# bacpop/sparrowhawk

Hardware: AMD Instinct MI355X
Metric: Gbases/s assembled, k=31 150bp reads (higher is better)
Workload: dtype u64

## Files before the change

### sparrowhawk_amd/csrc/graph_part.h

```cpp
#pragma once

struct MinScan {
    Nt32State first, last;
    uint32_t h_first, h_last;
    uint32_t min_wo_first;
    uint32_t min_wo_last;
    __device__ __forceinline__ uint32_t min_all() const { return min(min_wo_first, h_first); }
};

template <int W> __device__ __forceinline__ uint32_t km_base(const Kmer<W> &x, int k, int j) {
    return km_bits2<W>(x, 2 * (k - 1 - j));
}

template <int W> __device__ __forceinline__ MinScan km_min_scan(const Kmer<W> &x, int k, int gm) {
    MinScan r;
    Nt32State nt{0, 0};
    for (int j = 0; j < gm; j++) nt32_init_step(nt, km_base<W>(x, k, j), (unsigned)j);
    r.first = nt; r.h_first = nt32_canonical(nt);
    r.min_wo_first = 0xFFFFFFFFu; r.min_wo_last = r.h_first;
    const int w = k - gm + 1;
    uint32_t h = r.h_first;
    for (int q = 1; q < w; q++) {
        nt32_roll(nt, km_base<W>(x, k, q - 1), km_base<W>(x, k, q + gm - 1), (unsigned)gm);
        h = nt32_canonical(nt);
// ... 176 lines not shown
            uint32_t sz = gp_table_size(c);
            if (p >= GP) sz = 0;
            uint32_t si = sz, ci = c;
#pragma unroll
            for (int o = 1; o < 16; o <<= 1) {
                const uint32_t u = (uint32_t)__shfl_up((int)si, o), v = (uint32_t)__shfl_up((int)ci, o);
                if ((lane & 15) >= o) { si += u; ci += v; }
            }
            if (p < GP) { off[p] = run_off[e >> 4] + (si - sz); msk[p] = sz - 1u; roff[p] = run_roff[e >> 4] + (ci - c); }
        }
        for (int w = 0; w < 16; w++) { carry += wsum[w]; rcarry += rsum[w]; }
        __syncthreads();
    }
    if (threadIdx.x == 0) { *total = carry; roff[GP] = rcarry; }
}

__global__ __launch_bounds__(256) void k_gp_rows(const uint32_t *__restrict__ gp_of, uint32_t n,
                                                 const uint32_t *__restrict__ roff, uint32_t *__restrict__ cursor,
                                                 uint32_t *__restrict__ rows) {
    const int lane = threadIdx.x & 63;
    const uint32_t stride = gridDim.x * blockDim.x;
    const uint32_t n_round = (n + stride - 1) / stride * stride;
    for (uint32_t i = blockIdx.x * blockDim.x + threadIdx.x; i < n_round; i += stride) {
        const uint32_t p = i < n ? gp_of[i] : 0xFFFFFFFFu;
        const bool valid = p != 0xFFFFFFFFu;
        unsigned long long todo = __ballot(valid);
        int my_leader = lane; uint32_t rank = 0, gsize = 0;
        while (todo) {
            const int leader = __ffsll((long long)todo) - 1;
            const uint32_t lp = (uint32_t)__shfl((int)p, leader);
            const unsigned long long same = __ballot(p == lp) & todo;
            if (valid && p == lp) { my_leader = leader; rank = (uint32_t)__popcll(same & ((1ull << lane) - 1ull)); gsize = (uint32_t)__popcll(same); }
            todo &= ~same;
        }
        const uint32_t ro = valid ? roff[p] : 0u;
        uint32_t base = 0;
        if (valid && lane == my_leader) base = atomicAdd(&cursor[p], gsize);
        base = (uint32_t)__shfl((int)base, my_leader);
        if (valid) rows[ro + base + rank] = i;
    }
}

template <int W>
__global__ __launch_bounds__(256) void k_regroup_rows(KeyArr<W> keys, const uint32_t *__restrict__ cnt, const uint32_t *__restrict__ gp_of,
                                                      uint32_t *__restrict__ rows, uint32_t n, KeyArr<W> out_keys,
                                                      uint32_t *__restrict__ out_cnt, uint32_t *__restrict__ out_gp_of) {
    for (uint32_t r = blockIdx.x * blockDim.x + threadIdx.x; r < n; r += gridDim.x * blockDim.x) {
        const uint32_t i = rows[r];
        out_keys.store(r, keys.load(i));
        out_cnt[r] = cnt[i];
        out_gp_of[r] = gp_of[i];
        rows[r] = r;
    }
}

template <int W>
__device__ __forceinline__ uint32_t gt_lookup_in(const GraphTable &gt, const KeyArr<W> &keys, const Kmer<W> &q,
                                                 uint32_t p) {
    const uint64_t h = gt_hash<W>(q);
    const uint32_t fp = (uint32_t)(h >> 32);
    const unsigned long long base = gt.off[p];
    const uint32_t mask = gt.msk[p];
    uint32_t slot = (uint32_t)h & mask;
    for (uint32_t t = 0; t <= mask; t++) {
        const uint64_t e = gt.e[base + slot];
        if (e == EMPTY64) return NIL;
        if ((uint32_t)(e >> 32) == fp) {
            const uint32_t idx = (uint32_t)e;
            if (km_eq<W>(keys.load(idx), q)) return idx;
        }
        slot = (slot + 1) & mask;
    }
    return NIL;
}
template <int W>
__device__ __forceinline__ uint32_t gt_lookup(const GraphTable &gt, const KeyArr<W> &keys, const Kmer<W> &q, int k) {
    return gt_lookup_in<W>(gt, keys, q, gt_partition_of<W>(gt, q, k));
}

static constexpr uint32_t ADJ_LDS_SLOTS = 2048;
static constexpr uint32_t NB_MULTI = 0xFFFFFFFEu;
static constexpr uint32_t ADJ_LDS_SLOTS_RANGES = 4096;
static constexpr int ADJ_THREADS_RANGES = 512;

struct GpRows {
    const uint32_t *roff;
    const uint32_t *cnt;
    const uint32_t *rows;
    __device__ __forceinline__ uint32_t begin(uint32_t P) const { return roff[P]; }
    __device__ __forceinline__ uint32_t end(uint32_t P) const { return cnt ? roff[P] + cnt[P] : roff[P + 1]; }
    __device__ __forceinline__ uint32_t row(uint32_t r) const { return rows ? rows[r] : r; }
};

template <int W>
__device__ __forceinline__ Kmer<W> adj_candidate(const Kmer<W> &x, const Kmer<W> &rx, int k, uint32_t j, bool &o) {
    Kmer<W> s = x, rr = rx;
    if (j < 4) { km_push_back<W>(s, j, k); km_push_front<W>(rr, 3u - j, k); }
    else { km_push_front<W>(s, j - 4u, k); km_push_back<W>(rr, 3u - (j - 4u), k); }
    o = km_less<W>(rr, s);
    Kmer<W> c;
#pragma unroll
    for (int w = 0; w < W; w++) c.w[w] = o ? rr.w[w] : s.w[w];
    return c;
}

template <int W, uint32_t SLOTS, int NT>
__global__ __launch_bounds__(NT) void k_graph_local(KeyArr<W> keys, int k, GraphTable gt, GpRows gr,
                                                    uint8_t *__restrict__ adj, uint32_t *__restrict__ nb,
                                                    unsigned long long *__restrict__ queries, uint32_t *__restrict__ qcnt,
                                                    uint32_t *__restrict__ overflow, uint32_t lds_slots ,
                                                    uint8_t *__restrict__ alive, uint32_t *__restrict__ row_bits, uint32_t lowmask) {
    const unsigned gm = (unsigned)gt.gm;
    __shared__ uint2 lut[16];
    __shared__ uint64_t tab[SLOTS];
    __shared__ uint32_t tabi[W == 1 ? SLOTS : 1];
    __shared__ uint32_t q_fill;
    const uint32_t P = blockIdx.x;
    const bool ranges = gr.cnt != nullptr;
    const uint32_t r0 = gr.begin(P), r1 = gr.end(P);
    const uint32_t pmask = gt.msk[P];
    const bool in_lds = pmask < lds_slots;
    uint64_t *gtab = gt.e + gt.off[P];
    nt32_fill_lut(lut, gm);
    const Nt32State all_a = nt32_all_a(gt.gm);
    if (threadIdx.x == 0) q_fill = 0;
    constexpr bool KEYS_IN_LDS = W == 1;
    for (uint32_t t = threadIdx.x; t <= pmask; t += blockDim.x) {
        if (in_lds) tab[t] = EMPTY64;
        if (!in_lds || KEYS_IN_LDS) gtab[t] = EMPTY64;
    }
    __syncthreads();
    constexpr int KEEP = 4;
    static_assert(SLOTS <= 2u * KEEP * NT, "a partition whose table fits the LDS keeps its rows in registers");
    const bool keep = W <= 2 && (r1 - r0) <= (uint32_t)KEEP * NT;
    static_assert(KEEP == 4, "kept rows are four named registers");
    const uint32_t rt = r0 + threadIdx.x;
    const uint32_t i0 = (keep && rt < r1) ? gr.row(rt) : NIL, i1 = (keep && rt + NT < r1) ? gr.row(rt + NT) : NIL;
    const uint32_t i2 = (keep && rt + 2 * NT < r1) ? gr.row(rt + 2 * NT) : NIL, i3 = (keep && rt + 3 * NT < r1) ? gr.row(rt + 3 * NT) : NIL;
    const Kmer<W> k0 = i0 != NIL ? keys.load(i0) : km_zero<W>(), k1 = i1 != NIL ? keys.load(i1) : km_zero<W>();
    const Kmer<W> k2 = i2 != NIL ? keys.load(i2) : km_zero<W>(), k3 = i3 != NIL ? keys.load(i3) : km_zero<W>();
    auto kept_i = [=](uint32_t q) { return q == 0 ? i0 : (q == 1 ? i1 : (q == 2 ? i2 : i3)); };
    auto kept_key = [=](uint32_t q) {
        Kmer<W> r;
#pragma unroll
        for (int w = 0; w < W; w++) r.w[w] = q == 0 ? k0.w[w] : (q == 1 ? k1.w[w] : (q == 2 ? k2.w[w] : k3.w[w]));
        return r;
    };
    for (uint32_t r = r0 + threadIdx.x, q = 0; r < r1; r += blockDim.x, q++) {
        const uint32_t i = keep ? kept_i(q) : gr.row(r);
        const Kmer<W> key = keep ? kept_key(q) : keys.load(i);
        const uint64_t h = gt_hash<W>(key);
        const uint64_t entry = (h & 0xFFFFFFFF00000000ull) | (uint64_t)i;
        uint32_t slot = (uint32_t)h & pmask;
        bool done = false;
        for (uint32_t t = 0; t <= pmask; t++) {
            if (in_lds && KEYS_IN_LDS) {
                if (atomicCAS((unsigned long long *)&tab[slot], (unsigned long long)EMPTY64, (unsigned long long)key.w[0]) == EMPTY64) {
                    tabi[slot] = i; gtab[slot] = entry; done = true; break;
                }
            } else {
                unsigned long long *cell = in_lds ? (unsigned long long *)&tab[slot] : (unsigned long long *)&gtab[slot];
                if (atomicCAS(cell, (unsigned long long)EMPTY64, (unsigned long long)entry) == EMPTY64) { done = true; break; }
            }
            slot = (slot + 1) & pmask;
        }
        if (!done) *overflow = 1;
    }
    __syncthreads();
    if (ranges && threadIdx.x == NT - 1 && r1 > r0) {
        bool st = r0 == 0u;
        if (!st) st = ((km_min_scan_lut<W>(keys.load(r0 - 1u), k, gt.gm, lut, all_a).min_all() ^ P) & lowmask) != 0u;
        if (st) atomicOr(&row_bits[r0 >> 5], 1u << (r0 & 31u));
    }
    if (in_lds && !KEYS_IN_LDS) for (uint32_t t = threadIdx.x; t <= pmask; t += blockDim.x) gtab[t] = tab[t];
    {
        uint8_t *occ = gt.occ + (gt.off[P] >> 3);
        for (uint32_t t8 = threadIdx.x; t8 <= (pmask >> 3); t8 += blockDim.x) {
            uint32_t bits = 0;
#pragma unroll
            for (uint32_t b = 0; b < 8; b++) {
                const uint64_t e = in_lds ? tab[8u * t8 + b] : __hip_atomic_load(&gtab[8u * t8 + b], __ATOMIC_RELAXED, __HIP_MEMORY_SCOPE_AGENT);
                bits |= (e != EMPTY64 ? 1u : 0u) << b;
            }
            occ[t8] = (uint8_t)bits;
        }
    }
    unsigned long long *myq = queries + 8ull * r0;
    const int lane = threadIdx.x & 63;
    const uint32_t n_rows = r1 - r0;
    const uint32_t n_round = (n_rows + blockDim.x - 1) / blockDim.x * blockDim.x;
    for (uint32_t rr_ = threadIdx.x, q = 0; rr_ < n_round; rr_ += blockDim.x, q++) {
        const bool act = rr_ < n_rows;
        const uint32_t i = act ? (keep ? kept_i(q) : gr.row(r0 + rr_)) : 0u;
        Kmer<W> x = km_zero<W>(), rx = km_zero<W>();
        MinScan ms{};
        uint32_t out_b = 0, last_b = 0;
        if (act) {
            x = keep ? kept_key(q) : keys.load(i);
            rx = km_revcomp<W>(x, k);
            if (gt.scan) {
                const uint2 a = gt.scan[i], b = gt.scan[(size_t)gt.scan_n + i], c = gt.scan[2 * (size_t)gt.scan_n + i];
                ms.first.fh = a.x; ms.first.rh = a.y; ms.last.fh = b.x; ms.last.rh = b.y; ms.min_wo_first = c.x; ms.min_wo_last = c.y;
                ms.h_first = min(a.x, a.y); ms.h_last = min(b.x, b.y);
            } else ms = km_min_scan_lut<W>(x, k, gt.gm, lut, all_a);
            if (ranges && ((ms.min_all() & gt.gp_mask) != P)) *overflow = 2u;
            out_b = km_base<W>(x, k, k - (int)gm);
            last_b = km_base<W>(x, k, (int)gm - 1);
        }
        uint32_t a = 0, n_out = 0, n_in = 0, u_out = NIL, u_in = NIL;
#pragma unroll
        for (uint32_t j = 0; j < 8; j++) {
            bool remote = false; uint32_t p = 0, xowner = 0; bool cross = false;
            if (act) {
                const uint32_t hmin = j < 4 ? min(ms.min_wo_first, nt32_next_hash_lut(ms.last, out_b, j, lut))
                                            : min(ms.min_wo_last, nt32_prev_hash_lut(ms.first, j - 4u, last_b, lut));
                p = hmin & gt.gp_mask;
                if (gt.world > 1) { xowner = gt.owner_of(hmin); cross = xowner != gt.rank; }
                remote = cross || p != P || !in_lds;
                if (!remote) {
                    bool o; const Kmer<W> c = adj_candidate<W>(x, rx, k, j, o);
                    const uint64_t h = gt_hash<W>(c);
                    const uint32_t fp = (uint32_t)(h >> 32);
                    uint32_t slot = (uint32_t)h & pmask, idx = NIL;
                    for (uint32_t t = 0; t <= pmask; t++) {
                        const uint64_t e = tab[slot];
                        if (e == EMPTY64) break;
                        if constexpr (KEYS_IN_LDS) { if (e == c.w[0]) { idx = tabi[slot]; break; } }
                        else if ((uint32_t)(e >> 32) == fp && km_eq<W>(keys.load((uint32_t)e), c)) { idx = (uint32_t)e; break; }
                        slot = (slot + 1) & pmask;
                    }
                    (void)fp;
                    if (idx != NIL) {
                        a |= 1u << j;
                        if (j < 4) { n_out++; u_out = idx * 2u + (o ? 1u : 0u); }
                        else { n_in++; u_in = idx * 2u + (o ? 0u : 1u); }
                    }
                }
            }
            const unsigned long long m = __ballot(remote);
            if (m) {
                uint32_t base = 0;
                if (lane == 0) base = atomicAdd(&q_fill, (uint32_t)__popcll(m));
                base = (uint32_t)__shfl((int)base, 0);
                if (remote) myq[base + (uint32_t)__popcll(m & ((1ull << lane) - 1ull))] =
                    (unsigned long long)i | ((unsigned long long)j << 32) | ((unsigned long long)p << 35) |
                    (cross ? (1ull << 63) | ((unsigned long long)xowner << 52) : 0ull);
            }
        }
        if (act) {
            adj[i] = (uint8_t)a;
            if (alive) alive[i] = 1;
            uint2 v;
            v.x = n_out == 0 ? NIL : (n_out == 1 ? u_out : NB_MULTI);
            v.y = n_in == 0 ? NIL : (n_in == 1 ? u_in : NB_MULTI);
            *reinterpret_cast<uint2 *>(nb + 2ull * i) = v;
        }
    }
    __syncthreads();
    if (threadIdx.x == 0) qcnt[P] = q_fill;
}

template <int W>
__global__ __launch_bounds__(256) void k_graph_remote(KeyArr<W> keys, int k, GraphTable gt, GpRows gr,
                                                      const unsigned long long *__restrict__ queries,
                                                      const uint32_t *__restrict__ qcnt,
                                                      uint8_t *__restrict__ adj, uint32_t *__restrict__ nb) {
    const uint32_t P = blockIdx.x;
    const unsigned long long *myq = queries + 8ull * gr.begin(P);
    const uint32_t nq = qcnt[P];
    constexpr int U = W <= 2 ? 4 : (W <= 4 ? 2 : 1);
    for (uint32_t t0 = threadIdx.x; t0 < nq; t0 += blockDim.x * U) {
        unsigned long long q[U]; bool live[U];
#pragma unroll
        for (int u = 0; u < U; u++) {
            const uint32_t t = t0 + (uint32_t)u * blockDim.x;
            q[u] = t < nq ? myq[t] : ~0ull;
            live[u] = !(q[u] >> 63);
        }
        Kmer<W> x[U]; unsigned long long tbase[U]; uint32_t tmask[U];
#pragma unroll
        for (int u = 0; u < U; u++) {
            const uint32_t i = (uint32_t)q[u], p = (uint32_t)(q[u] >> 35) & 0x1FFFFu;
            x[u] = live[u] ? keys.load(i) : km_zero<W>();
            tbase[u] = live[u] ? gt.off[p] : 0ull;
            tmask[u] = live[u] ? gt.msk[p] : 0u;
        }
        Kmer<W> c[U]; bool o[U]; uint32_t fp[U], slot[U]; uint64_t e[U];
#pragma unroll
        for (int u = 0; u < U; u++) {
            const uint32_t j = (uint32_t)(q[u] >> 32) & 7u;
            const Kmer<W> rx = km_revcomp<W>(x[u], k);
            c[u] = adj_candidate<W>(x[u], rx, k, j, o[u]);
            const uint64_t h = gt_hash<W>(c[u]);
            fp[u] = (uint32_t)(h >> 32); slot[u] = (uint32_t)h & tmask[u];
        }
        bool taken[U];
#pragma unroll
        for (int u = 0; u < U; u++) {
            const unsigned long long s = tbase[u] + slot[u];
            taken[u] = live[u] && ((gt.occ[s >> 3] >> (s & 7u)) & 1u);
        }
#pragma unroll
        for (int u = 0; u < U; u++) e[u] = taken[u] ? gt.e[tbase[u] + slot[u]] : EMPTY64;
        Kmer<W> cand[U]; bool want[U];
#pragma unroll
        for (int u = 0; u < U; u++) {
            want[u] = e[u] != EMPTY64 && (uint32_t)(e[u] >> 32) == fp[u];
            cand[u] = want[u] ? keys.load((uint32_t)e[u]) : km_zero<W>();
        }
#pragma unroll
        for (int u = 0; u < U; u++) {
            if (!live[u]) continue;
            uint32_t idx = NIL;
            if (want[u] && km_eq<W>(cand[u], c[u])) idx = (uint32_t)e[u];
            else if (e[u] != EMPTY64) {
                uint32_t s = (slot[u] + 1u) & tmask[u];
                for (uint32_t t = 1; t <= tmask[u]; t++) {
                    const uint64_t ee = gt.e[tbase[u] + s];
                    if (ee == EMPTY64) break;
                    if ((uint32_t)(ee >> 32) == fp[u] && km_eq<W>(keys.load((uint32_t)ee), c[u])) { idx = (uint32_t)ee; break; }
                    s = (s + 1u) & tmask[u];
                }
            }
            if (idx == NIL) continue;
            const uint32_t i = (uint32_t)q[u], j = (uint32_t)(q[u] >> 32) & 7u;
            atomicOr((uint32_t *)adj + (i >> 2), (1u << j) << (8 * (i & 3u)));
            const uint32_t v = j < 4 ? idx * 2u + (o[u] ? 1u : 0u) : idx * 2u + (o[u] ? 0u : 1u);
            uint32_t *dst = nb + 2ull * i + (j < 4 ? 0 : 1);
            if (atomicCAS(dst, NIL, v) != NIL) atomicExch(dst, NB_MULTI);
        }
    }
}

__device__ __forceinline__ uint32_t rev4(uint32_t n) {
    return ((n & 1) << 3) | ((n & 2) << 1) | ((n & 4) >> 1) | ((n & 8) >> 3);
}
__device__ __forceinline__ uint32_t outmask_of(uint32_t adjbyte, uint32_t o) {
    return o ? rev4(adjbyte >> 4) : (adjbyte & 15u);
}

template <int W> struct Graph {
    KeyArr<W> keys;
    const uint32_t *cnt;
    uint8_t *adj;
    GraphTable gt;
    const uint32_t *nb;
    int k;
    uint32_t n;
    uint32_t xref = 0;
    __device__ __forceinline__ uint32_t outmask(uint32_t v) const { return outmask_of(adj[v >> 1], v & 1); }
    __device__ __forceinline__ uint32_t outdeg(uint32_t v) const { return __popc(outmask(v)); }
    __device__ __forceinline__ uint32_t indeg(uint32_t v) const { return __popc(outmask(v ^ 1)); }
    __device__ __forceinline__ Kmer<W> seq(uint32_t v) const {
        Kmer<W> x = keys.load(v >> 1);
        return (v & 1) ? km_revcomp<W>(x, k) : x;
    }
    __device__ __forceinline__ uint32_t follow(uint32_t v, uint32_t b) const {
        Kmer<W> s = seq(v);
        km_push_back<W>(s, b, k);
        int o; Kmer<W> c = km_canonical<W>(s, k, o);
        uint32_t idx = gt_lookup<W>(gt, keys, c, k);
        return idx == NIL ? NIL : idx * 2 + (uint32_t)o;
    }
    __device__ __forceinline__ uint32_t only_out(uint32_t v) const {
        const uint32_t c = nb[v];
        if (c < NB_MULTI) return c;
        return follow(v, (uint32_t)__ffs((int)outmask(v)) - 1);
    }
};

struct TipRec { uint32_t start, junction, len, next; unsigned long long sum; };

template <int W>
__global__ __launch_bounds__(256) void k_tip_candidates(Graph<W> g, const uint8_t *__restrict__ alive,
                                                        uint32_t *__restrict__ cand,
                                                        unsigned int *__restrict__ n_cand,
                                                        uint2 *__restrict__ init_tip_head ,
                                                        uint8_t *__restrict__ init_mark ) {
    const int lane = threadIdx.x & 63;
    const uint32_t stride = gridDim.x * blockDim.x;
    const uint32_t n_round = (g.n + stride - 1) / stride * stride;
    for (uint32_t i = blockIdx.x * blockDim.x + threadIdx.x; i < n_round; i += stride) {
        uint32_t a = 0; bool al = false;
        if (i < g.n) {
            a = g.adj[i]; al = alive[i] != 0;
            if (init_tip_head) { uint2 nil; nil.x = NIL; nil.y = NIL; init_tip_head[i] = nil; init_mark[i] = 0; }
        }
#pragma unroll
        for (uint32_t o = 0; o < 2; o++) {
            const bool p = al && __popc(outmask_of(a, o ^ 1u)) == 0 && __popc(outmask_of(a, o)) == 1;
            const unsigned long long m = __ballot(p);
            if (!m) continue;
            unsigned int base = 0;
            if (lane == 0) base = atomicAdd(n_cand, (unsigned int)__popcll(m));
            base = __shfl(base, 0);
            if (p) cand[base + __popcll(m & ((1ull << lane) - 1ull))] = 2u * i + o;
        }
    }
}

template <int W>
__global__ __launch_bounds__(256) void k_tip_walk(Graph<W> g, const uint32_t *__restrict__ cand,
                                                  const unsigned int *__restrict__ n_cand_p, TipRec *__restrict__ tips,
                                                  unsigned int *__restrict__ n_tips,
                                                  uint32_t *__restrict__ tip_head) {
    const uint32_t T_TIP = 2u * (uint32_t)g.k;
    const uint32_t n_cand = *n_cand_p;
    for (uint32_t c = blockIdx.x * blockDim.x + threadIdx.x; c < n_cand; c += gridDim.x * blockDim.x) {
        const uint32_t v = cand[c];
        uint32_t cur = v, len = 1, J = NIL;
        unsigned long long sum = g.cnt[v >> 1];
        uint32_t a_cur = g.adj[cur >> 1], nb_cur = g.nb[cur];
// ... 211 lines not shown
```

### sparrowhawk_amd/csrc/pipeline.hip

```cpp
#include <hip/hip_runtime.h>
#include <hipcub/hipcub.hpp>
#include <thread>
#include <stdint.h>
#include <stdio.h>
#include <stdlib.h>
#include <string.h>
#include <algorithm>
#include <atomic>
#include <chrono>
#include <map>
#include <memory>
#include <mutex>
#include <string>
#include <vector>

#include "kmer.h"
#include "pipeline.h"
#include "shard_comm.h"
#include "unitig_graph.h"

namespace shk {

#define HIPCHK(call)                                                                      \
    do {                                                                                  \
// ... 1194 lines not shown
        have_parts_ = n_runs != 0;
        const uint64_t rows_hint = d_recv_w ? 2 * total_recs + (1u << 16) : std::max<uint64_t>(1u << 16, total_recs);
        if (int rc = run_count_partitions(run_view_, n_owned, emit_threshold, ekeys_, ecnt_, n_emitted_, histo, inst,
                                          rows_hint, ms, err)) return rc;
        times_.add("count_kernel", ms);
        total_instances_ = inst;
        for (int i = 0; i < 500; i++) { histo_[i] = histo[i]; n_distinct_ += histo[i]; }
        return 0;
    }

    int shard_rows(uint32_t threshold, const void **keys_soa, const void **cnt, uint64_t *n, std::string &err) override {
        if (int rc = filter(threshold, err)) return rc;
        for (int j = 0; j < W; j++) keys_soa[j] = skeys_[j].p;
        *cnt = scnt_.p; *n = n_solid_;
        return 0;
    }

    int shard_set_solid(const void *const *keys_soa, const void *cnt, uint64_t n, const uint64_t histo[500],
                        uint64_t total_instances, std::string &err) override {
        if (n >= 0x7FFFFFFFull) { err = "too many solid k-mers for 32-bit node ids"; return -1; }
        DevBuf<uint64_t> nk[W]; DevBuf<uint32_t> nc;
        for (int j = 0; j < W; j++) {
            if (int rc = nk[j].alloc(n, err)) return rc;
            if (n) HIPCHK(hipMemcpyAsync(nk[j].p, keys_soa[j], n * 8, hipMemcpyDeviceToDevice, stream_));
        }
        if (int rc = nc.alloc(n, err)) return rc;
        if (n) HIPCHK(hipMemcpyAsync(nc.p, cnt, n * 4, hipMemcpyDeviceToDevice, stream_));
        WAIT_STREAM();
        for (int j = 0; j < W; j++) skeys_[j].swap(nk[j]);
        scnt_.swap(nc);
        n_solid_ = n; total_instances_ = total_instances; n_distinct_ = 0; er_ok_ = false;
        for (int i = 0; i < 500; i++) { histo_[i] = histo[i]; n_distinct_ += histo[i]; }
        graph_ready_ = false;
        return 0;
    }

    Graph<W> graph_view() {
        Graph<W> g;
        for (int j = 0; j < W; j++) g.keys.w[j] = skeys_[j].p;
        g.cnt = scnt_.p; g.adj = adj_.p; g.nb = nb_.p; g.k = k_;
        g.gt.e = gt_.p; g.gt.occ = gt_occ_.p; g.gt.scan = gt_scan_.p; g.gt.scan_n = gt_scan_.p ? (uint32_t)n_solid_ : 0u; g.gt.off = gt_off_.p; g.gt.msk = gt_msk_.p; g.gt.gp_mask = gp_ - 1u; g.gt.gm = part_m(k_);
        g.n = (uint32_t)n_solid_;
        if (sh_active_) {
            g.gt.cp_mask = sh_P_ - 1u; g.gt.world = sh_world_; g.gt.rank = sh_rank_;
            g.gt.world_inv = (uint32_t)((0x100000000ull + sh_world_ - 1u) / sh_world_);
            g.xref = XREF;
        }
        return g;
    }

    int build_graph(std::string &err) override {
        const uint64_t n = n_solid_;
        for (int j = 0; j < W; j++) tkeys_[j].release();
        tcnt_.release(); tstate_.release(); tslots_ = 0;
        recs_.release(); fill_.release(); run_off_.release(); run_cnt_.release(); shard_recv_ = nullptr; batches_.clear();
        const uint64_t regroup_env = env_u64("SHK_REGROUP_ROWS", 2);
        const uint64_t range_rows = env_u64("SHK_GRAPH_RANGE_ROWS", ADJ_LDS_SLOTS_RANGES * 3 / 8);
        const bool ranges = er_ok_ && er_rows_ == n && n && !sh_active_ && !rows_scattered_ && regroup_env != 1 &&
                            n <= (uint64_t)er_groups_ * range_rows &&
                            getenv("SHK_GP_ROWS") == nullptr && env_u64("SHK_GRAPH_RANGES", 1) != 0;
        er_ok_ = false;
        gp_ = 64;
        const uint64_t gp_rows_target = env_u64("SHK_GP_ROWS", 640);
        const uint64_t n_for_gp = sh_active_ ? n_solid_global_ : n;
        while (gp_ < GP_MAX && (uint64_t)gp_ * gp_rows_target < n_for_gp) gp_ <<= 1;
        if (ranges) gp_ = er_groups_;
        gt_slots_ = 4 * n + 8ull * gp_;
        if (int rc = gt_.alloc(gt_slots_, err)) return rc;
        if (int rc = gt_occ_.alloc(gt_slots_ / 8 + 8, err)) return rc;
        gt_scan_.release();
        if (!ranges && n && n <= (64ull << 20) && env_u64("SHK_KEEP_SCAN", 1)) if (int rc = gt_scan_.alloc(3 * n, err)) return rc;
        DevBuf<uint32_t> gp_of, gp_cnt, gp_roff, gp_rows, gp_n;
        if (ranges) {
            gt_off_.swap(er_off_); gt_msk_.swap(er_msk_); gp_roff.swap(er_start_); gp_n.swap(er_cnt_);
            er_off_.release(); er_msk_.release(); er_start_.release(); er_cnt_.release();
        } else {
            if (int rc = gt_off_.alloc(gp_, err)) return rc;
            if (int rc = gt_msk_.alloc(gp_, err)) return rc;
            if (int rc = gp_of.alloc(n, err)) return rc;
            if (int rc = gp_roff.alloc(gp_ + 1, err)) return rc;
            if (int rc = gp_rows.alloc(n, err)) return rc;
        }
        if (int rc = gp_cnt.alloc(gp_, err)) return rc;
        DevBuf<unsigned long long> queries;
        if (int rc = queries.alloc(8 * n + 8, err)) return rc;
        if (int rc = adj_.alloc((n + 8) & ~3ull, err)) return rc;
        if (keep_stages_) if (int rc = adj0_.alloc(n, err)) return rc;
        if (int rc = nb_.alloc(2 * n + 2, err)) return rc;
        if (int rc = alive_.alloc(n, err)) return rc;
        if (int rc = row_starts_.alloc(((n + 63) / 64) * 2 + 2, err)) return rc;
        if (ranges) HIPCHK(fill2_async(row_starts_.p, row_starts_.bytes, 0u, ctl_.p, CTL_WORDS * sizeof(unsigned long long), 0u, stream_));
        else HIPCHK(fill2_async(gp_cnt.p, (size_t)gp_ * 4, 0u, ctl_.p, CTL_WORDS * sizeof(unsigned long long), 0u, stream_));
        if (n || sh_active_) {
            Graph<W> g = graph_view();
            const uint32_t lowmask = std::min<uint32_t>(gp_, 256u) - 1u;
            if (ranges) {
                EvTimer t(stream_, stage_timers_);
                t.stop_later("graph_table_kernel", pending_timers_);
                EvTimer t2(stream_, stage_timers_);
                const GpRows gr{gp_roff.p, gp_n.p, nullptr};
                const uint32_t lds_slots = (uint32_t)std::min<uint64_t>(env_u64("SHK_GRAPH_LDS_SLOTS", ADJ_LDS_SLOTS_RANGES), ADJ_LDS_SLOTS_RANGES);
                hipLaunchKernelGGL((k_graph_local<W, ADJ_LDS_SLOTS_RANGES, ADJ_THREADS_RANGES>), dim3(gp_), dim3(ADJ_THREADS_RANGES), 0, stream_,
                                   g.keys, k_, g.gt, gr, adj_.p, nb_.p, queries.p, gp_cnt.p, (uint32_t *)(ctl_.p + 1), lds_slots,
                                   alive_.p, row_starts_.p, lowmask);
                hipLaunchKernelGGL(k_graph_remote<W>, dim3(gp_), dim3(256), 0, stream_, g.keys, k_, g.gt, gr, queries.p,
                                   gp_cnt.p, adj_.p, nb_.p);
                HIPCHK(hipGetLastError());
                t2.stop_later("adjacency_kernel", pending_timers_);
                times_.add("graph_partitions_from_counting_x1", 1.0);
            } else {
                EvTimer t(stream_, stage_timers_);
                hipLaunchKernelGGL(k_gp_count<W>, dim3(grid_for(n)), dim3(256), 0, stream_, g.keys, (uint32_t)n, k_, g.gt,
                                   gp_of.p, gp_cnt.p);
                hipLaunchKernelGGL(k_gp_scan, dim3(1), dim3(1024), 0, stream_, gp_cnt.p, gp_, gt_off_.p, gt_msk_.p, gp_roff.p,
                                   ctl_.p + 2);
                hipLaunchKernelGGL(k_gp_rows, dim3(grid_for(n)), dim3(256), 0, stream_, gp_of.p, (uint32_t)n, gp_roff.p, gp_cnt.p,
                                   gp_rows.p);
                HIPCHK(hipGetLastError());
                if (n && (regroup_env == 1 || (regroup_env == 2 && rows_scattered_))) {
                    DevBuf<uint64_t> nk[W]; DevBuf<uint32_t> nc, ngp;
                    for (int j = 0; j < W; j++) if (int rc = nk[j].alloc(n, err)) return rc;
                    if (int rc = nc.alloc(n, err)) return rc;
                    if (int rc = ngp.alloc(n, err)) return rc;
                    KeyArr<W> out_keys; for (int j = 0; j < W; j++) out_keys.w[j] = nk[j].p;
                    hipLaunchKernelGGL(k_regroup_rows<W>, dim3(grid_for(n)), dim3(256), 0, stream_, g.keys, scnt_.p, gp_of.p, gp_rows.p, (uint32_t)n,
                                       out_keys, nc.p, ngp.p);
                    HIPCHK(hipGetLastError());
                    WAIT_STREAM();
                    for (int j = 0; j < W; j++) skeys_[j].swap(nk[j]);
                    scnt_.swap(nc); gp_of.swap(ngp);
                    gt_scan_.release();
                    g = graph_view();
                    times_.add("graph_rows_regrouped_x1", 1.0);
                }
                hipLaunchKernelGGL(k_row_starts, dim3(grid_for(n)), dim3(256), 0, stream_, gp_of.p, (uint32_t)n, lowmask,
                                   row_starts_.p, alive_.p);
                t.stop_later("graph_table_kernel", pending_timers_);
                EvTimer t2(stream_, stage_timers_);
                const GpRows gr{gp_roff.p, nullptr, gp_rows.p};
                hipLaunchKernelGGL((k_graph_local<W, ADJ_LDS_SLOTS, 256>), dim3(gp_), dim3(256), 0, stream_, g.keys, k_, g.gt, gr,
                                   adj_.p, nb_.p, queries.p, gp_cnt.p, (uint32_t *)(ctl_.p + 1), ADJ_LDS_SLOTS,
                                   (uint8_t *)nullptr, (uint32_t *)nullptr, 0u);
                hipLaunchKernelGGL(k_graph_remote<W>, dim3(gp_), dim3(256), 0, stream_, g.keys, k_, g.gt, gr, queries.p,
                                   gp_cnt.p, adj_.p, nb_.p);
                HIPCHK(hipGetLastError());
                t2.stop_later("adjacency_kernel", pending_timers_);
                times_.add("graph_partitions_cut_x1", 1.0);
            }
            if (sh_active_ && sh_world_ > 1) {
                HIPCHK(fill2_async(ctl_.p + 13, 8, 0u, nullptr, 0, 0u, stream_));
                hipLaunchKernelGGL(k_xq_total, dim3(gp_), dim3(256), 0, stream_, gp_roff.p, queries.p, gp_cnt.p, (unsigned int *)(ctl_.p + 13));
                unsigned int n_x = 0;
                if (int rc = read_ctl(n_x, 13, err)) return rc;
                xq_n_ = n_x;
                if (int rc = xq_dest_.alloc(n_x, err)) return rc;
                if (int rc = xq_pay_.alloc((size_t)n_x * (W + 1), err)) return rc;
                if (int rc = xq_meta_.alloc(n_x, err)) return rc;
                if (n_x) {
                    HIPCHK(fill2_async(ctl_.p + 13, 8, 0u, nullptr, 0, 0u, stream_));
                    hipLaunchKernelGGL(k_xq_stage<W>, dim3(gp_), dim3(256), 0, stream_, g.keys, k_, gp_roff.p, queries.p, gp_cnt.p,
                                       (unsigned int *)(ctl_.p + 13), n_x, xq_dest_.p, xq_pay_.p, xq_meta_.p);
                    HIPCHK(hipGetLastError());
                }
            }
            if (keep_stages_) HIPCHK(hipMemcpyAsync(adj0_.p, adj_.p, n, hipMemcpyDeviceToDevice, stream_));
            graph_check_pending_ = true;
            if (sh_active_) {
                HIPCHK(hipMemcpyAsync(mbox64() + MB_CTL, ctl_.p, 3 * 8, hipMemcpyDeviceToHost, stream_));
// ... 1140 lines not shown
```

### sparrowhawk_amd/csrc/shard_graph.h

```cpp
#pragma once

static constexpr uint32_t XREF = 0x80000000u;
static constexpr int ROUTE_CH = 4096;
static constexpr uint32_t ROUTE_MAX_WORLD = 256;

__global__ __launch_bounds__(256) void k_route_count(const uint32_t *__restrict__ dest, uint32_t n, unsigned long long *__restrict__ counts) {
    __shared__ uint32_t h[ROUTE_MAX_WORLD];
    h[threadIdx.x] = 0;
    __syncthreads();
    for (uint32_t i = blockIdx.x * blockDim.x + threadIdx.x; i < n; i += gridDim.x * blockDim.x) {
        const uint32_t d = dest[i];
        if (d < ROUTE_MAX_WORLD) atomicAdd(&h[d], 1u);
    }
    __syncthreads();
    if (h[threadIdx.x]) atomicAdd(&counts[threadIdx.x], (unsigned long long)h[threadIdx.x]);
}
template <int PW>
__global__ __launch_bounds__(256) void k_route_pack(const uint32_t *__restrict__ dest, const uint64_t *__restrict__ pay, uint32_t n,
                                                    unsigned long long *__restrict__ cursors, uint64_t *__restrict__ send,
                                                    uint32_t *__restrict__ sidx) {
    __shared__ uint32_t h[ROUTE_MAX_WORLD];
    __shared__ unsigned long long base[ROUTE_MAX_WORLD];
    h[threadIdx.x] = 0;
    __syncthreads();
    const uint32_t i0 = blockIdx.x * ROUTE_CH, i1 = min(n, i0 + (uint32_t)ROUTE_CH);
    for (uint32_t i = i0 + threadIdx.x; i < i1; i += blockDim.x) { const uint32_t d = dest[i]; if (d < ROUTE_MAX_WORLD) atomicAdd(&h[d], 1u); }
    __syncthreads();
    if (h[threadIdx.x]) base[threadIdx.x] = atomicAdd(&cursors[threadIdx.x], (unsigned long long)h[threadIdx.x]);
    __syncthreads();
    h[threadIdx.x] = 0;
    __syncthreads();
    for (uint32_t i = i0 + threadIdx.x; i < i1; i += blockDim.x) {
        const uint32_t d = dest[i];
        if (d >= ROUTE_MAX_WORLD) continue;
        const unsigned long long at = base[d] + atomicAdd(&h[d], 1u);
#pragma unroll
        for (int j = 0; j < PW; j++) send[at * PW + j] = pay[(uint64_t)i * PW + j];
        if (sidx) sidx[i] = (uint32_t)at;
    }
}

__global__ __launch_bounds__(256) void k_xq_total(const uint32_t *__restrict__ roff, const unsigned long long *__restrict__ queries,
                                                  const uint32_t *__restrict__ qcnt, unsigned int *__restrict__ total) {
    const unsigned long long *myq = queries + 8ull * roff[blockIdx.x];
    const uint32_t nq = qcnt[blockIdx.x];
    uint32_t mine = 0;
    for (uint32_t t = threadIdx.x; t < nq; t += blockDim.x) mine += (uint32_t)(myq[t] >> 63);
    for (int o = 32; o > 0; o >>= 1) mine += __shfl_down(mine, o);
    if ((threadIdx.x & 63) == 0 && mine) atomicAdd(total, mine);
}
template <int W>
__global__ __launch_bounds__(256) void k_xq_stage(KeyArr<W> keys, int k, const uint32_t *__restrict__ roff,
                                                  const unsigned long long *__restrict__ queries, const uint32_t *__restrict__ qcnt,
                                                  unsigned int *__restrict__ n_staged, uint32_t cap,
                                                  uint32_t *__restrict__ dest, uint64_t *__restrict__ pay ,
                                                  unsigned long long *__restrict__ meta) {
    __shared__ uint32_t blk_n, blk_base;
    const uint32_t P = blockIdx.x;
    const unsigned long long *myq = queries + 8ull * roff[P];
    const uint32_t nq = qcnt[P];
    if (threadIdx.x == 0) blk_n = 0;
    __syncthreads();
    uint32_t mine = 0;
    for (uint32_t t = threadIdx.x; t < nq; t += blockDim.x) mine += (uint32_t)(myq[t] >> 63);
    if (mine) atomicAdd(&blk_n, mine);
    __syncthreads();
    if (threadIdx.x == 0) blk_base = blk_n ? atomicAdd(n_staged, blk_n) : 0u;
    __syncthreads();
    if (!blk_n) return;
    if (threadIdx.x == 0) blk_n = 0;
    __syncthreads();
    for (uint32_t t = threadIdx.x; t < nq; t += blockDim.x) {
        const unsigned long long q = myq[t];
        if (!(q >> 63)) continue;
        const uint32_t at = blk_base + atomicAdd(&blk_n, 1u);
        if (at >= cap) continue;
        const uint32_t i = (uint32_t)q, j = (uint32_t)(q >> 32) & 7u, p = (uint32_t)(q >> 35) & 0x1FFFFu, d = (uint32_t)(q >> 52) & 0xFFu;
        const Kmer<W> x = keys.load(i);
        const Kmer<W> rx = km_revcomp<W>(x, k);
        bool o; const Kmer<W> c = adj_candidate<W>(x, rx, k, j, o);
        dest[at] = d;
#pragma unroll
        for (int w = 0; w < W; w++) pay[(uint64_t)at * (W + 1) + w] = c.w[w];
        pay[(uint64_t)at * (W + 1) + W] = p;
        meta[at] = (unsigned long long)i | ((unsigned long long)j << 32) | ((unsigned long long)(o ? 1u : 0u) << 35) | ((unsigned long long)d << 36);
    }
}
template <int W>
__global__ __launch_bounds__(256) void k_xq_answer(KeyArr<W> keys, GraphTable gt, const uint64_t *__restrict__ recv, uint64_t n_recv,
                                                   unsigned long long gbase, unsigned long long *__restrict__ ans) {
    for (uint64_t t = (uint64_t)blockIdx.x * blockDim.x + threadIdx.x; t < n_recv; t += (uint64_t)gridDim.x * blockDim.x) {
        Kmer<W> c;
#pragma unroll
        for (int w = 0; w < W; w++) c.w[w] = recv[t * (W + 1) + w];
        const uint32_t p = (uint32_t)recv[t * (W + 1) + W] & gt.gp_mask;
        const uint32_t idx = gt_lookup_in<W>(gt, keys, c, p);
        ans[t] = idx == NIL ? ~0ull : gbase + idx;
    }
}
__global__ __launch_bounds__(256) void k_xq_apply(const unsigned long long *__restrict__ meta, const uint32_t *__restrict__ sidx,
                                                  const unsigned long long *__restrict__ ans, uint32_t n_items,
                                                  uint8_t *__restrict__ adj, uint32_t *__restrict__ nb,
                                                  unsigned long long *__restrict__ xnb) {
    for (uint32_t t = blockIdx.x * blockDim.x + threadIdx.x; t < n_items; t += gridDim.x * blockDim.x) {
        const unsigned long long a = ans[sidx[t]];
        xnb[t] = ~0ull;
        if (a == ~0ull) continue;
        const unsigned long long m = meta[t];
        const uint32_t i = (uint32_t)m, j = (uint32_t)(m >> 32) & 7u, o = (uint32_t)(m >> 35) & 1u;
        atomicOr((uint32_t *)adj + (i >> 2), (1u << j) << (8 * (i & 3u)));
        xnb[t] = a * 2ull + (j < 4 ? o : (o ^ 1u));
        uint32_t *slot = nb + 2ull * i + (j < 4 ? 0 : 1);
        if (atomicCAS(slot, NIL, XREF | t) != NIL) atomicExch(slot, NB_MULTI);
    }
}

__global__ __launch_bounds__(256) void k_hl_stage(const uint8_t *__restrict__ adj, const uint32_t *__restrict__ nb, uint32_t n_nodes,
                                                  const unsigned long long *__restrict__ xnb, const unsigned long long *__restrict__ meta,
                                                  unsigned long long gbase, uint32_t *__restrict__ dest, uint64_t *__restrict__ pay ) {
    const uint32_t total = 2u * n_nodes;
    for (uint32_t v = blockIdx.x * blockDim.x + threadIdx.x; v < total; v += gridDim.x * blockDim.x) {
        uint32_t d = NIL;
        const uint32_t u = nb[v];
        if ((u & XREF) && u < NB_MULTI && __popc(outmask_of(adj[v >> 1], v & 1u)) == 1) {
            const uint32_t t = u & ~XREF;
            d = (uint32_t)(meta[t] >> 36) & 0xFFu;
            pay[2ull * v] = xnb[t];
            pay[2ull * v + 1] = 2ull * gbase + v;
        }
        dest[v] = d;
    }
}
__global__ __launch_bounds__(256) void k_hl_apply(const uint64_t *__restrict__ recv, uint64_t n_recv, unsigned long long gbase, uint32_t n_nodes,
                                                  const uint8_t *__restrict__ adj, uint32_t *__restrict__ xpred, uint32_t *__restrict__ flags) {
    for (uint64_t t = (uint64_t)blockIdx.x * blockDim.x + threadIdx.x; t < n_recv; t += (uint64_t)gridDim.x * blockDim.x) {
        const unsigned long long w = recv[2 * t];
        if (w < 2ull * gbase || w - 2ull * gbase >= 2ull * n_nodes) { flags[0] = 1; continue; }
        const uint32_t wl = (uint32_t)(w - 2ull * gbase);
        if (__popc(outmask_of(adj[wl >> 1], (wl & 1u) ^ 1u)) == 1) xpred[wl] = (uint32_t)t;
    }
}

__global__ __launch_bounds__(256) void k_lchain_stage(const HeadRec *__restrict__ heads, uint32_t n_heads, const uint32_t *__restrict__ xpred,
                                                      const uint64_t *__restrict__ hl_recv, const unsigned long long *__restrict__ gbases,
                                                      uint32_t world, SegRec *__restrict__ segs, uint32_t *__restrict__ dest,
                                                      uint64_t *__restrict__ pay ) {
    for (uint32_t s = blockIdx.x * blockDim.x + threadIdx.x; s < n_heads; s += gridDim.x * blockDim.x) {
        const HeadRec h = heads[s];
        SegRec r; r.node = s; r.next_spl = NIL; r.len = (uint32_t)h.len; r.last = h.tail_node; r.sum = h.kc; r.head = 0; r.pad = 0;
        uint32_t d = NIL;
        if (h.circ) r.head = HEAD_ORPHAN;
        else {
            const bool has_pred = xpred[h.head_node] != NIL;
            if (!has_pred) r.head = HEAD_LINEAR;
            const uint32_t ref = xpred[h.tail_node ^ 1u];
            if (ref != NIL) {
// ... 197 lines not shown
```

Before: 175.7.

## Halve remote graph edge queries via symmetric edge insertion and carried candidate hash

```diff
diff --git a/sparrowhawk_amd/csrc/graph_part.h b/sparrowhawk_amd/csrc/graph_part.h
--- a/sparrowhawk_amd/csrc/graph_part.h
+++ b/sparrowhawk_amd/csrc/graph_part.h
@@ -282,6 +282,9 @@
 static constexpr uint32_t NB_MULTI = 0xFFFFFFFEu;
 static constexpr uint32_t ADJ_LDS_SLOTS_RANGES = 4096;
 static constexpr int ADJ_THREADS_RANGES = 512;
+typedef ulonglong2 GraphQuery;
+static constexpr uint32_t GQ_PER_ROW = 8;
+static constexpr int GQ_O_BIT = 60, GQ_MB_BIT = 61;
 
 struct GpRows {
     const uint32_t *roff;
@@ -307,7 +310,7 @@
 template <int W, uint32_t SLOTS, int NT>
 __global__ __launch_bounds__(NT) void k_graph_local(KeyArr<W> keys, int k, GraphTable gt, GpRows gr,
                                                     uint8_t *__restrict__ adj, uint32_t *__restrict__ nb,
-                                                    unsigned long long *__restrict__ queries, uint32_t *__restrict__ qcnt,
+                                                    GraphQuery *__restrict__ queries, uint32_t *__restrict__ qcnt,
                                                     uint32_t *__restrict__ overflow, uint32_t lds_slots ,
                                                     uint8_t *__restrict__ alive, uint32_t *__restrict__ row_bits, uint32_t lowmask) {
     const unsigned gm = (unsigned)gt.gm;
@@ -385,7 +388,7 @@
             occ[t8] = (uint8_t)bits;
         }
     }
-    unsigned long long *myq = queries + 8ull * r0;
+    GraphQuery *myq = queries + (unsigned long long)GQ_PER_ROW * r0;
     const int lane = threadIdx.x & 63;
     const uint32_t n_rows = r1 - r0;
     const uint32_t n_round = (n_rows + blockDim.x - 1) / blockDim.x * blockDim.x;
@@ -410,41 +413,54 @@
         uint32_t a = 0, n_out = 0, n_in = 0, u_out = NIL, u_in = NIL;
 #pragma unroll
         for (uint32_t j = 0; j < 8; j++) {
-            bool remote = false; uint32_t p = 0, xowner = 0; bool cross = false;
+            bool ask = false, o = false; uint32_t p = 0, xowner = 0; bool cross = false;
+            unsigned long long carried = 0;
             if (act) {
                 const uint32_t hmin = j < 4 ? min(ms.min_wo_first, nt32_next_hash_lut(ms.last, out_b, j, lut))
                                             : min(ms.min_wo_last, nt32_prev_hash_lut(ms.first, j - 4u, last_b, lut));
                 p = hmin & gt.gp_mask;
                 if (gt.world > 1) { xowner = gt.owner_of(hmin); cross = xowner != gt.rank; }
-                remote = cross || p != P || !in_lds;
-                if (!remote) {
-                    bool o; const Kmer<W> c = adj_candidate<W>(x, rx, k, j, o);
-                    const uint64_t h = gt_hash<W>(c);
-                    const uint32_t fp = (uint32_t)(h >> 32);
-                    uint32_t slot = (uint32_t)h & pmask, idx = NIL;
-                    for (uint32_t t = 0; t <= pmask; t++) {
-                        const uint64_t e = tab[slot];
-                        if (e == EMPTY64) break;
-                        if constexpr (KEYS_IN_LDS) { if (e == c.w[0]) { idx = tabi[slot]; break; } }
-                        else if ((uint32_t)(e >> 32) == fp && km_eq<W>(keys.load((uint32_t)e), c)) { idx = (uint32_t)e; break; }
-                        slot = (slot + 1) & pmask;
-                    }
-                    (void)fp;
-                    if (idx != NIL) {
-                        a |= 1u << j;
-                        if (j < 4) { n_out++; u_out = idx * 2u + (o ? 1u : 0u); }
-                        else { n_in++; u_in = idx * 2u + (o ? 0u : 1u); }
+                const bool remote = cross || p != P || !in_lds;
+                if (cross) ask = true;
+                else {
+                    const Kmer<W> c = adj_candidate<W>(x, rx, k, j, o);
+                    if (!remote) {
+                        const uint64_t h = gt_hash<W>(c);
+                        const uint32_t fp = (uint32_t)(h >> 32);
+                        uint32_t slot = (uint32_t)h & pmask, idx = NIL;
+                        for (uint32_t t = 0; t <= pmask; t++) {
+                            const uint64_t e = tab[slot];
+                            if (e == EMPTY64) break;
+                            if constexpr (KEYS_IN_LDS) { if (e == c.w[0]) { idx = tabi[slot]; break; } }
+                            else if ((uint32_t)(e >> 32) == fp && km_eq<W>(keys.load((uint32_t)e), c)) { idx = (uint32_t)e; break; }
+                            slot = (slot + 1) & pmask;
+                        }
+                        (void)fp;
+                        if (idx != NIL) {
+                            a |= 1u << j;
+                            if (j < 4) { n_out++; u_out = idx * 2u + (o ? 1u : 0u); }
+                            else { n_in++; u_in = idx * 2u + (o ? 0u : 1u); }
+                        }
+                    } else if (!km_less<W>(c, x)) {
+                        ask = true;
+                        if constexpr (W == 1) carried = c.w[0]; else carried = gt_hash<W>(c);
                     }
                 }
             }
-            const unsigned long long m = __ballot(remote);
+            const unsigned long long m = __ballot(ask);
             if (m) {
                 uint32_t base = 0;
                 if (lane == 0) base = atomicAdd(&q_fill, (uint32_t)__popcll(m));
                 base = (uint32_t)__shfl((int)base, 0);
-                if (remote) myq[base + (uint32_t)__popcll(m & ((1ull << lane) - 1ull))] =
-                    (unsigned long long)i | ((unsigned long long)j << 32) | ((unsigned long long)p << 35) |
-                    (cross ? (1ull << 63) | ((unsigned long long)xowner << 52) : 0ull);
+                if (ask) {
+                    const uint32_t mb = j < 4 ? km_first_base<W>(x, k) : km_last_base<W>(x);
+                    GraphQuery q;
+                    q.x = (unsigned long long)i | ((unsigned long long)j << 32) | ((unsigned long long)p << 35) |
+                          (cross ? (1ull << 63) | ((unsigned long long)xowner << 52)
+                                 : ((unsigned long long)(o ? 1u : 0u) << GQ_O_BIT) | ((unsigned long long)mb << GQ_MB_BIT));
+                    q.y = carried;
+                    myq[base + (uint32_t)__popcll(m & ((1ull << lane) - 1ull))] = q;
+                }
             }
         }
         if (act) {
@@ -460,38 +476,41 @@
     if (threadIdx.x == 0) qcnt[P] = q_fill;
 }
 
+__device__ __forceinline__ void graph_add_edge_end(uint8_t *adj, uint32_t *nb, uint32_t node, uint32_t bit, uint32_t side, uint32_t v) {
+    atomicOr((uint32_t *)adj + (node >> 2), (1u << bit) << (8 * (node & 3u)));
+    uint32_t *dst = nb + 2ull * node + side;
+    if (atomicCAS(dst, NIL, v) != NIL) atomicExch(dst, NB_MULTI);
+}
 template <int W>
 __global__ __launch_bounds__(256) void k_graph_remote(KeyArr<W> keys, int k, GraphTable gt, GpRows gr,
-                                                      const unsigned long long *__restrict__ queries,
+                                                      const GraphQuery *__restrict__ queries,
                                                       const uint32_t *__restrict__ qcnt,
                                                       uint8_t *__restrict__ adj, uint32_t *__restrict__ nb) {
     const uint32_t P = blockIdx.x;
-    const unsigned long long *myq = queries + 8ull * gr.begin(P);
+    const GraphQuery *myq = queries + (unsigned long long)GQ_PER_ROW * gr.begin(P);
     const uint32_t nq = qcnt[P];
     constexpr int U = W <= 2 ? 4 : (W <= 4 ? 2 : 1);
     for (uint32_t t0 = threadIdx.x; t0 < nq; t0 += blockDim.x * U) {
-        unsigned long long q[U]; bool live[U];
+        GraphQuery q[U]; bool live[U];
 #pragma unroll
         for (int u = 0; u < U; u++) {
             const uint32_t t = t0 + (uint32_t)u * blockDim.x;
-            q[u] = t < nq ? myq[t] : ~0ull;
-            live[u] = !(q[u] >> 63);
-        }
-        Kmer<W> x[U]; unsigned long long tbase[U]; uint32_t tmask[U];
+            q[u].x = ~0ull; q[u].y = 0ull;
+            if (t < nq) q[u] = myq[t];
+            live[u] = !(q[u].x >> 63);
+        }
+        unsigned long long tbase[U]; uint32_t tmask[U];
 #pragma unroll
         for (int u = 0; u < U; u++) {
-            const uint32_t i = (uint32_t)q[u], p = (uint32_t)(q[u] >> 35) & 0x1FFFFu;
-            x[u] = live[u] ? keys.load(i) : km_zero<W>();
+            const uint32_t i = (uint32_t)q[u].x, p = (uint32_t)(q[u].x >> 35) & 0x1FFFFu;
             tbase[u] = live[u] ? gt.off[p] : 0ull;
             tmask[u] = live[u] ? gt.msk[p] : 0u;
         }
-        Kmer<W> c[U]; bool o[U]; uint32_t fp[U], slot[U]; uint64_t e[U];
+        uint32_t fp[U], slot[U]; uint64_t e[U];
 #pragma unroll
         for (int u = 0; u < U; u++) {
-            const uint32_t j = (uint32_t)(q[u] >> 32) & 7u;
-            const Kmer<W> rx = km_revcomp<W>(x[u], k);
-            c[u] = adj_candidate<W>(x[u], rx, k, j, o[u]);
-            const uint64_t h = gt_hash<W>(c[u]);
+            uint64_t h = q[u].y;
+            if constexpr (W == 1) { Kmer<W> c; c.w[0] = q[u].y; h = gt_hash<W>(c); }
             fp[u] = (uint32_t)(h >> 32); slot[u] = (uint32_t)h & tmask[u];
         }
         bool taken[U];
@@ -502,32 +521,44 @@
         }
 #pragma unroll
         for (int u = 0; u < U; u++) e[u] = taken[u] ? gt.e[tbase[u] + slot[u]] : EMPTY64;
-        Kmer<W> cand[U]; bool want[U];
+        Kmer<W> cand[U], x[U]; bool want[U];
 #pragma unroll
         for (int u = 0; u < U; u++) {
             want[u] = e[u] != EMPTY64 && (uint32_t)(e[u] >> 32) == fp[u];
             cand[u] = want[u] ? keys.load((uint32_t)e[u]) : km_zero<W>();
+            x[u] = (W > 1 && e[u] != EMPTY64) ? keys.load((uint32_t)q[u].x) : km_zero<W>();
         }
 #pragma unroll
         for (int u = 0; u < U; u++) {
-            if (!live[u]) continue;
+            if (!live[u] || e[u] == EMPTY64) continue;
+            const uint32_t i = (uint32_t)q[u].x, j = (uint32_t)(q[u].x >> 32) & 7u;
+            const bool o = (q[u].x >> GQ_O_BIT) & 1ull;
+            Kmer<W> c = km_zero<W>(); bool have_c = W == 1;
+            auto make_c = [&]() {
+                if constexpr (W == 1) c.w[0] = q[u].y;
+                else if (!have_c) { bool o2; c = adj_candidate<W>(x[u], km_revcomp<W>(x[u], k), k, j, o2); have_c = true; }
+            };
+            if (want[u]) make_c();
             uint32_t idx = NIL;
-            if (want[u] && km_eq<W>(cand[u], c[u])) idx = (uint32_t)e[u];
-            else if (e[u] != EMPTY64) {
+            if (want[u] && km_eq<W>(cand[u], c)) idx = (uint32_t)e[u];
+            else {
                 uint32_t s = (slot[u] + 1u) & tmask[u];
                 for (uint32_t t = 1; t <= tmask[u]; t++) {
                     const uint64_t ee = gt.e[tbase[u] + s];
                     if (ee == EMPTY64) break;
-                    if ((uint32_t)(ee >> 32) == fp[u] && km_eq<W>(keys.load((uint32_t)ee), c[u])) { idx = (uint32_t)ee; break; }
+                    if ((uint32_t)(ee >> 32) == fp[u]) { make_c(); if (km_eq<W>(keys.load((uint32_t)ee), c)) { idx = (uint32_t)ee; break; } }
                     s = (s + 1u) & tmask[u];
                 }
             }
             if (idx == NIL) continue;
-            const uint32_t i = (uint32_t)q[u], j = (uint32_t)(q[u] >> 32) & 7u;
-            atomicOr((uint32_t *)adj + (i >> 2), (1u << j) << (8 * (i & 3u)));
-            const uint32_t v = j < 4 ? idx * 2u + (o[u] ? 1u : 0u) : idx * 2u + (o[u] ? 0u : 1u);
-            uint32_t *dst = nb + 2ull * i + (j < 4 ? 0 : 1);
-            if (atomicCAS(dst, NIL, v) != NIL) atomicExch(dst, NB_MULTI);
+            const uint32_t mb = (uint32_t)(q[u].x >> GQ_MB_BIT) & 3u;
+            if (j < 4) {
+                graph_add_edge_end(adj, nb, i, j, 0u, idx * 2u + (o ? 1u : 0u));
+                if (idx != i) graph_add_edge_end(adj, nb, idx, o ? 3u - mb : 4u + mb, o ? 0u : 1u, 2u * i + 1u);
+            } else {
+                graph_add_edge_end(adj, nb, i, j, 1u, idx * 2u + (o ? 0u : 1u));
+                if (idx != i) graph_add_edge_end(adj, nb, idx, o ? 4u + (3u - mb) : mb, o ? 1u : 0u, 2u * i);
+            }
         }
     }
 }
diff --git a/sparrowhawk_amd/csrc/pipeline.hip b/sparrowhawk_amd/csrc/pipeline.hip
--- a/sparrowhawk_amd/csrc/pipeline.hip
+++ b/sparrowhawk_amd/csrc/pipeline.hip
@@ -1300,8 +1300,8 @@
             if (int rc = gp_rows.alloc(n, err)) return rc;
         }
         if (int rc = gp_cnt.alloc(gp_, err)) return rc;
-        DevBuf<unsigned long long> queries;
-        if (int rc = queries.alloc(8 * n + 8, err)) return rc;
+        DevBuf<GraphQuery> queries;
+        if (int rc = queries.alloc(GQ_PER_ROW * n + 8, err)) return rc;
         if (int rc = adj_.alloc((n + 8) & ~3ull, err)) return rc;
         if (keep_stages_) if (int rc = adj0_.alloc(n, err)) return rc;
         if (int rc = nb_.alloc(2 * n + 2, err)) return rc;
diff --git a/sparrowhawk_amd/csrc/shard_graph.h b/sparrowhawk_amd/csrc/shard_graph.h
--- a/sparrowhawk_amd/csrc/shard_graph.h
+++ b/sparrowhawk_amd/csrc/shard_graph.h
@@ -40,29 +40,29 @@
     }
 }
 
-__global__ __launch_bounds__(256) void k_xq_total(const uint32_t *__restrict__ roff, const unsigned long long *__restrict__ queries,
+__global__ __launch_bounds__(256) void k_xq_total(const uint32_t *__restrict__ roff, const GraphQuery *__restrict__ queries,
                                                   const uint32_t *__restrict__ qcnt, unsigned int *__restrict__ total) {
-    const unsigned long long *myq = queries + 8ull * roff[blockIdx.x];
+    const GraphQuery *myq = queries + (unsigned long long)GQ_PER_ROW * roff[blockIdx.x];
     const uint32_t nq = qcnt[blockIdx.x];
     uint32_t mine = 0;
-    for (uint32_t t = threadIdx.x; t < nq; t += blockDim.x) mine += (uint32_t)(myq[t] >> 63);
+    for (uint32_t t = threadIdx.x; t < nq; t += blockDim.x) mine += (uint32_t)(myq[t].x >> 63);
     for (int o = 32; o > 0; o >>= 1) mine += __shfl_down(mine, o);
     if ((threadIdx.x & 63) == 0 && mine) atomicAdd(total, mine);
 }
 template <int W>
 __global__ __launch_bounds__(256) void k_xq_stage(KeyArr<W> keys, int k, const uint32_t *__restrict__ roff,
-                                                  const unsigned long long *__restrict__ queries, const uint32_t *__restrict__ qcnt,
+                                                  const GraphQuery *__restrict__ queries, const uint32_t *__restrict__ qcnt,
                                                   unsigned int *__restrict__ n_staged, uint32_t cap,
                                                   uint32_t *__restrict__ dest, uint64_t *__restrict__ pay ,
                                                   unsigned long long *__restrict__ meta) {
     __shared__ uint32_t blk_n, blk_base;
     const uint32_t P = blockIdx.x;
-    const unsigned long long *myq = queries + 8ull * roff[P];
+    const GraphQuery *myq = queries + (unsigned long long)GQ_PER_ROW * roff[P];
     const uint32_t nq = qcnt[P];
     if (threadIdx.x == 0) blk_n = 0;
     __syncthreads();
     uint32_t mine = 0;
-    for (uint32_t t = threadIdx.x; t < nq; t += blockDim.x) mine += (uint32_t)(myq[t] >> 63);
+    for (uint32_t t = threadIdx.x; t < nq; t += blockDim.x) mine += (uint32_t)(myq[t].x >> 63);
     if (mine) atomicAdd(&blk_n, mine);
     __syncthreads();
     if (threadIdx.x == 0) blk_base = blk_n ? atomicAdd(n_staged, blk_n) : 0u;
@@ -71,7 +71,7 @@
     if (threadIdx.x == 0) blk_n = 0;
     __syncthreads();
     for (uint32_t t = threadIdx.x; t < nq; t += blockDim.x) {
-        const unsigned long long q = myq[t];
+        const unsigned long long q = myq[t].x;
         if (!(q >> 63)) continue;
         const uint32_t at = blk_base + atomicAdd(&blk_n, 1u);
         if (at >= cap) continue;
```

After: 177.5, median of 4. About the same (+1.0%).
